# Ipsedo/MARLClassification

Hardware: NVIDIA B200
Metric: image_episodes_per_sec (higher is better)
Workload: dtype tf32x3

## Files before the change

marlclassification_b200/csrc/gemm_tc.cu:

```cuda
#include <cuda.h>
#include <stdlib.h>

#include "common.cuh"
#include "tc.cuh"

namespace marlc {

constexpr int BM = 128;
constexpr int BK = 32;
constexpr int UMMA_K = 8;
constexpr int TC_THREADS = 192;
constexpr int TC_THREADS_X3 = 320;
constexpr int TC_SPLITTERS = TC_THREADS_X3 - 64;
#define TC_SPLIT_GROUPS(stages) (((stages) % 2 == 0) ? 2 : 1)
constexpr int TC_MAX_CHAIN = 4096;

typedef CUresult (*EncodeTiledFn)(CUtensorMap*, CUtensorMapDataType, cuuint32_t, void*, const cuuint64_t*,
                                  const cuuint64_t*, const cuuint32_t*, const cuuint32_t*, CUtensorMapInterleave,
                                  CUtensorMapSwizzle, CUtensorMapL2promotion, CUtensorMapFloatOOBfill);
static EncodeTiledFn get_encode() {
    static EncodeTiledFn fn = nullptr;
    if (!fn) {
        void* p = nullptr;
        cudaDriverEntryPointQueryResult q;
        if (cudaGetDriverEntryPoint("cuTensorMapEncodeTiled", &p, cudaEnableDefault, &q) == cudaSuccess &&
            q == cudaDriverEntryPointSuccess)
            fn = (EncodeTiledFn)p;
    }
    return fn;
}

static int make_map(CUtensorMap* m, const float* ptr, long inner, long rows, long slabs, long ld, long slab_stride,
                    int box_rows, bool mn_major = false, int box_slabs = 1) {
    EncodeTiledFn enc = get_encode();
    MARLC_CHECK(enc, "cuTensorMapEncodeTiled not available");
    cuuint64_t dims[3] = {(cuuint64_t)inner, (cuuint64_t)rows, (cuuint64_t)slabs};
// ... 95 lines not shown
__device__ __forceinline__ float ex2_ftz(float x) { float y; asm("ex2.approx.ftz.f32 %0, %1;" : "=f"(y) : "f"(x)); return y; }
__device__ __forceinline__ float rcp_ftz(float x) { float y; asm("rcp.approx.ftz.f32 %0, %1;" : "=f"(y) : "f"(x)); return y; }
__device__ __forceinline__ float sigmoid_of_scaled(float t) { return rcp_ftz(1.0f + ex2_ftz(t)); }
__device__ __forceinline__ float tanh_of_scaled(float t) { return fmaf(2.0f, rcp_ftz(1.0f + ex2_ftz(t)), -1.0f); }
__device__ __forceinline__ float fast_tanh(float x) { return tanh_of_scaled(2.0f * NEG_LOG2E * x); }

__device__ __forceinline__ uint64_t make_desc(uint32_t saddr, uint32_t lbo_bytes, uint32_t sbo_bytes, uint32_t layout_type) {
    return (uint64_t)((saddr >> 4) & 0x3FFF) | ((uint64_t)((lbo_bytes >> 4) & 0x3FFF) << 16) |
           ((uint64_t)((sbo_bytes >> 4) & 0x3FFF) << 32) | (1ull << 46) | ((uint64_t)layout_type << 61);
}

enum { EPI_STORE = 0, EPI_LSTM = 1 };

struct TcKernelParams {
    CUtensorMap a1, b1, a2, b2;
    CUtensorMap a1l, b1l, a2l, b2l;
    CUtensorMap cmap;
    int c_tma;
    int ksplit;
    int a_lo_g, b_lo_g;
    int nk1, nk2;
    int slab_a1, slab_b1, slab_a2, slab_b2;
    int M, N;
    float* C;
    long ldc;
    const float* bias;
    const float* bias2;
    int accumulate, splits;
    const float* c_prev;
    float* c_new;
    float* h_new;
    float* h_new_lo;
    float* gates;
    int n_hidden;
};
constexpr int TC_MAX_GROUP = 3;
struct TcKernelGroup {
    TcKernelParams p[TC_MAX_GROUP];
    int zofs[TC_MAX_GROUP + 1];
    int count;
    int trig;
};

template <int BN, int STAGES, bool X3 = false, int KS = 1>
struct TcSmem {
    static constexpr int A_SUB = BM * BK * 4;
    static constexpr int B_SUB = BN * BK * 4;
    static constexpr int A_BYTES = KS * A_SUB;
    static constexpr int B_BYTES = KS * B_SUB;
    static constexpr int BYTES = STAGES * (A_BYTES + B_BYTES) * (X3 ? 2 : 1) + 1024;
};


template <int BN, bool A_MN, bool B_MN, int EPI, int STAGES, int PI, bool X3, int KS>
__device__ __forceinline__ void tc_gemm_body(const TcKernelGroup& pp, const int split) {
    using S = TcSmem<BN, STAGES, X3, KS>;
    extern __shared__ uint8_t smem_raw[];
    uint8_t* smem = (uint8_t*)(((uintptr_t)smem_raw + 1023) & ~(uintptr_t)1023);
    constexpr int stages = STAGES;
    uint8_t* sA = smem;
    uint8_t* sB = smem + stages * S::A_BYTES;
    constexpr int LO_OFF = stages * (S::A_BYTES + S::B_BYTES);
    __shared__ __align__(8) uint64_t full_bar[STAGES];
    __shared__ __align__(8) uint64_t empty_bar[STAGES];
    __shared__ __align__(8) uint64_t split_bar[STAGES];
    __shared__ __align__(8) uint64_t tmem_full_bar;
    __shared__ uint32_t tmem_base_smem;
    __shared__ float s_bias[8][BN];

    const TcKernelParams& p = pp.p[PI];
    const int warp = threadIdx.x >> 5, lane = threadIdx.x & 31;
#ifdef MARLC_TC_TRACE
    __shared__ long long trace[12];
    const bool tr = blockIdx.x == 0 && blockIdx.y == 0 && blockIdx.z == 0;
    const long long t_entry = clock64();
#define TC_TRACE(i) do { if (tr) trace[i] = clock64() - t_entry; } while (0)
#else
#define TC_TRACE(i) do { } while (0)
#endif
    const int m0 = blockIdx.y * BM;
    const int ksp = (EPI == EPI_LSTM && p.ksplit > 1) ? p.ksplit : 1;
    const int n_tile = ksp > 1 ? blockIdx.x / ksp : blockIdx.x;
    const int kslice = ksp > 1 ? blockIdx.x % ksp : 0;
    if (m0 >= p.M || n_tile * BN >= p.N) return;
    const int nkb = p.nk1 + p.nk2;
    int kb_begin = 0, kb_end = nkb;
    if (EPI == EPI_STORE && p.splits > 1) {
        const int per = (nkb + p.splits - 1) / p.splits;
        kb_begin = split * per;
        kb_end = min(nkb, kb_begin + per);
    }
    if (ksp > 1) {
        const int per = (nkb + ksp - 1) / ksp;
        kb_begin = kslice * per;
        kb_end = min(nkb, kb_begin + per);
    }
    const int my_kb = max(0, kb_end - kb_begin);
    constexpr int TMEM_COLS = BN < 32 ? 32 : BN;

    if (warp == 0 && lane == 0) {
        auto pf = [](const CUtensorMap* m) { asm volatile("prefetch.tensormap [%0];" ::"l"((uint64_t)m) : "memory"); };
        pf(&p.a1); pf(&p.b1);
        if (p.nk2 > 0) { pf(&p.a2); pf(&p.b2); }
        if (X3 && p.a_lo_g) { pf(&p.a1l); if (p.nk2 > 0) pf(&p.a2l); }
        if (X3 && p.b_lo_g) { pf(&p.b1l); if (p.nk2 > 0) pf(&p.b2l); }
        if (EPI == EPI_STORE && p.c_tma) pf(&p.cmap);
    }
    if (threadIdx.x == 32) {
        for (int s = 0; s < stages; ++s) {
            mbar_init(&full_bar[s], 1); mbar_init(&empty_bar[s], 1);
            mbar_init(&split_bar[s], TC_SPLITTERS / TC_SPLIT_GROUPS(STAGES));
        }
        mbar_init(&tmem_full_bar, 1);
        asm volatile("fence.mbarrier_init.release.cluster;" ::: "memory");
    }
    if (warp == 1) {
        asm volatile("tcgen05.alloc.cta_group::1.sync.aligned.shared::cta.b32 [%0], %1;" ::"r"(smem_u32(&tmem_base_smem)),
                     "r"(TMEM_COLS));
        asm volatile("tcgen05.relinquish_alloc_permit.cta_group::1.sync.aligned;");
    }
    tc_fence_before();
    __syncthreads();
    tc_fence_after();
    const uint32_t tmem_base = tmem_base_smem;
    pdl_wait();
    if (threadIdx.x == 0) TC_TRACE(0);
    if (ksp > 1) asm volatile("barrier.cluster.arrive.release;" ::: "memory");

    if (warp == 0) {
// ... 64 lines not shown
                    if (X3) {
                        const uint64_t lo = (uint64_t)((LO_OFF >> 4) & 0x3FFF);
                        umma_tf32(tmem_base, ad + lo, bd, idesc, 1u);
                        umma_tf32(tmem_base, ad, bd + lo, idesc, 1u);
                    }
                }
                }
                umma_commit(&empty_bar[s]);
            }
            umma_commit(&tmem_full_bar);
            TC_TRACE(3);
        }
    } else {
        const int q = warp & 3;
        const int m = m0 + 32 * q + lane;
        constexpr int HU_E = BN / 4;
        const bool epi8 = EPI == EPI_LSTM && X3 && HU_E >= 32 && ksp == 1 && p.a_lo_g && p.b_lo_g;
        const bool epi_warp = warp < 6 || epi8;
        const int jb_begin = (epi8 && warp >= 6) ? HU_E / 2 : 0;
        const int jb_end = epi8 ? (warp >= 6 ? HU_E : HU_E / 2) : HU_E;
        float cp_pref[8];
        if (epi_warp) {
            float* sb = s_bias[warp - 2];
            if (EPI == EPI_STORE) {
                const bool first_split0 = (p.splits <= 1) || (split == 0);
                for (int j = lane; j < BN; j += 32) {
                    const int n = n_tile * BN + j;
                    float b = 0.f;
                    if (first_split0 && n < p.N) {
                        if (p.bias) b += __ldg(p.bias + n);
                        if (p.bias2) b += __ldg(p.bias2 + n);
                    }
                    sb[j] = b;
                }
            } else {
                constexpr int HU = BN / 4;
                const int n = p.n_hidden, j0 = n_tile * HU;
                for (int j = lane; j < BN; j += 32) {
                    const int g = j / HU, col = g * n + j0 + (j - g * HU);
                    sb[j] = (__ldg(p.bias + col) + __ldg(p.bias2 + col)) * (g == 2 ? 2.0f * NEG_LOG2E : NEG_LOG2E);
                }
                if (m < p.M) {
                    const long off = (long)m * n + j0 + jb_begin;
                    const float4 c0 = *reinterpret_cast<const float4*>(p.c_prev + off);
                    const float4 c1 = *reinterpret_cast<const float4*>(p.c_prev + off + 4);
                    cp_pref[0] = c0.x; cp_pref[1] = c0.y; cp_pref[2] = c0.z; cp_pref[3] = c0.w;
                    cp_pref[4] = c1.x; cp_pref[5] = c1.y; cp_pref[6] = c1.z; cp_pref[7] = c1.w;
                }
            }
            __syncwarp();
        }
        if (X3) {
            constexpr int NGRP = TC_SPLIT_GROUPS(STAGES);
            constexpr int GRP = TC_SPLITTERS / NGRP;
            const int t = (threadIdx.x - 64) % GRP, grp = (threadIdx.x - 64) / GRP;
            const bool split_a = !p.a_lo_g, split_b = !p.b_lo_g;
            for (int i = grp; (split_a || split_b) && i < my_kb; i += NGRP) {
                const int s = i % stages, ph = (i / stages) & 1;
                mbar_wait(&full_bar[s], ph);
                float4* a_hi = reinterpret_cast<float4*>(sA + s * S::A_BYTES);
                float4* b_hi = reinterpret_cast<float4*>(sB + s * S::B_BYTES);
                float4* a_lo = reinterpret_cast<float4*>(sA + s * S::A_BYTES + LO_OFF);
                float4* b_lo = reinterpret_cast<float4*>(sB + s * S::B_BYTES + LO_OFF);
                auto lo_of = [](float x) { return x - __uint_as_float(__float_as_uint(x) & 0xFFFFE000u); };
#pragma unroll 4
                for (int v = t; split_a && v < S::A_BYTES / 16; v += GRP) {
                    const float4 x = a_hi[v];
                    a_lo[v] = make_float4(lo_of(x.x), lo_of(x.y), lo_of(x.z), lo_of(x.w));
                }
#pragma unroll 4
                for (int v = t; split_b && v < S::B_BYTES / 16; v += GRP) {
                    const float4 x = b_hi[v];
                    b_lo[v] = make_float4(lo_of(x.x), lo_of(x.y), lo_of(x.z), lo_of(x.w));
                }
                asm volatile("fence.proxy.async.shared::cta;" ::: "memory");
                asm volatile("mbarrier.arrive.shared::cta.b64 _, [%0];" ::"r"(smem_u32(&split_bar[s])) : "memory");
            }
        }
        if (epi_warp) {
        int e_M = p.M, e_N = p.N, e_mode = p.splits > 1 ? 2 : (p.accumulate ? 1 : 0);
        long e_ldc = p.ldc;
        float* e_C = p.C;
        asm volatile("" : "+r"(e_M), "+r"(e_N), "+r"(e_mode), "+l"(e_ldc), "+l"(e_C));
        mbar_wait(&tmem_full_bar, 0);
        tc_fence_after();
        if (warp == 2 && lane == 0) TC_TRACE(4);
        const uint32_t trow = tmem_base + ((uint32_t)(32 * q) << 16);
        if (EPI == EPI_STORE) {
            constexpr int PITCH = BN + 4;
            static_assert(EPI != EPI_STORE || 4 * 32 * PITCH * 4 <= S::BYTES - 1024, "epilogue staging tile does not fit in the ring");
            float* stg = reinterpret_cast<float*>(smem) + q * 32 * PITCH;
            const int nbase = n_tile * BN;
            const bool vec = ((e_ldc & 3) == 0) && (((uintptr_t)e_C & 15) == 0);
            if (p.c_tma) {
                constexpr int BOXES = BN / 32;
                const uint32_t box0 = smem_u32(smem) + (uint32_t)(q * BOXES) * 4096u;
#pragma unroll 1
                for (int c0 = 0; c0 < BN; c0 += 32) {
                    uint32_t r[32];
                    if (my_kb > 0) { TMEM_LD32(trow + c0, r); tmem_ld_wait(); }
                    else {
#pragma unroll
                        for (int j = 0; j < 32; ++j) r[j] = 0u;
                    }
                    const float* sb = s_bias[warp - 2] + c0;
                    const uint32_t rowb = box0 + (uint32_t)(c0 >> 5) * 4096u + (uint32_t)lane * 128u;
#pragma unroll
                    for (int j = 0; j < 32; j += 4) {
                        const uint32_t dst = rowb + (uint32_t)(((j >> 2) ^ (lane & 7)) << 4);
                        asm volatile("st.shared.v4.f32 [%0], {%1, %2, %3, %4};" ::"r"(dst),
                                     "f"(__uint_as_float(r[j]) + sb[j]), "f"(__uint_as_float(r[j + 1]) + sb[j + 1]),
                                     "f"(__uint_as_float(r[j + 2]) + sb[j + 2]), "f"(__uint_as_float(r[j + 3]) + sb[j + 3])
                                     : "memory");
                    }
                }
                asm volatile("fence.proxy.async.shared::cta;" ::: "memory");
                __syncwarp();
                if (warp == 2 && lane == 0) TC_TRACE(6);
                if (lane == 0 && m0 + 32 * q < e_M) {
#pragma unroll 1
                    for (int b = 0; b < BOXES; ++b) {
                        const int cn = nbase + 32 * b;
                        if (cn >= e_N) break;
                        const uint32_t src = box0 + (uint32_t)b * 4096u;
                        if (e_mode == 0)
                            asm volatile("cp.async.bulk.tensor.2d.global.shared::cta.bulk_group [%0, {%2, %3}], [%1];" ::"l"(
                                             (uint64_t)&p.cmap), "r"(src), "r"(cn), "r"(m0 + 32 * q) : "memory");
                        else
                            asm volatile("cp.reduce.async.bulk.tensor.2d.global.shared::cta.add.tile.bulk_group [%0, {%2, %3}], [%1];" ::"l"(
                                             (uint64_t)&p.cmap), "r"(src), "r"(cn), "r"(m0 + 32 * q) : "memory");
                    }
                    asm volatile("cp.async.bulk.commit_group;" ::: "memory");
                    asm volatile("cp.async.bulk.wait_group.read 0;" ::: "memory");
                }
            } else {
            const uint32_t stg_s = smem_u32(stg);
#pragma unroll 1
            for (int c0 = 0; c0 < BN; c0 += 32) {
                uint32_t r[32];
                if (my_kb > 0) { TMEM_LD32(trow + c0, r); tmem_ld_wait(); }
                else {
#pragma unroll
                    for (int j = 0; j < 32; ++j) r[j] = 0u;
                }
                const float* sb = s_bias[warp - 2] + c0;
#pragma unroll
                for (int j = 0; j < 32; j += 4) {
                    const float4 v = make_float4(__uint_as_float(r[j]) + sb[j], __uint_as_float(r[j + 1]) + sb[j + 1],
                                                 __uint_as_float(r[j + 2]) + sb[j + 2], __uint_as_float(r[j + 3]) + sb[j + 3]);
                    asm volatile("st.shared.v4.f32 [%0], {%1, %2, %3, %4};" ::"r"(stg_s + (uint32_t)(lane * PITCH + c0 + j) * 4),
                                 "f"(v.x), "f"(v.y), "f"(v.z), "f"(v.w) : "memory");
                }
            }
            __syncwarp();
            constexpr int LPR = BN / 4;
            constexpr int RPI = 32 / LPR;
            const int rr = lane / LPR, c4 = (lane % LPR) * 4;
            const int n = nbase + c4;
            const bool full4 = vec && n + 4 <= e_N;
            if (n < e_N) {
#pragma unroll 1
                for (int r0 = 0; r0 < 32; r0 += RPI) {
                    const int row = r0 + rr, mrow = m0 + 32 * q + row;
                    if (mrow >= e_M) break;
                    float4 v;
                    asm volatile("ld.shared.v4.f32 {%0, %1, %2, %3}, [%4];" : "=f"(v.x), "=f"(v.y), "=f"(v.z), "=f"(v.w)
                                 : "r"(stg_s + (uint32_t)(row * PITCH + c4) * 4));
                    float* crow = e_C + (long)mrow * e_ldc + n;
#ifdef MARLC_TC_NOSTORE
                    if (v.x == 123.456f) crow[0] = v.y;
                    continue;
#endif
#ifdef MARLC_TC_TRACE
                    if (warp == 2 && lane == 0 && r0 == RPI * 2) TC_TRACE(7);
#endif
                    if (full4) {
                        if (e_mode == 2) {
                            atomicAdd(reinterpret_cast<float4*>(crow), v);
                        } else {
                            if (e_mode == 1) {
                                const float4 o = *reinterpret_cast<const float4*>(crow);
                                v.x += o.x; v.y += o.y; v.z += o.z; v.w += o.w;
                            }
                            *reinterpret_cast<float4*>(crow) = v;
                        }
                    } else {
                        const float vv[4] = {v.x, v.y, v.z, v.w};
#pragma unroll
                        for (int j = 0; j < 4; ++j) {
                            if (n + j >= e_N) break;
                            if (e_mode == 2) atomicAdd(crow + j, vv[j]);
                            else crow[j] = e_mode == 1 ? crow[j] + vv[j] : vv[j];
                        }
                    }
                }
            }
            }
        } else {
            constexpr int HU = BN / 4;
            const int n = p.n_hidden, j0 = n_tile * HU;
            constexpr int PPITCH = BN + 4;
            float* part = reinterpret_cast<float*>(smem + (S::BYTES - 1024));
            if (ksp > 1) asm volatile("barrier.cluster.wait.acquire;" ::: "memory");
            if (ksp > 1 && kslice != 0) {
                uint32_t remote;
                asm volatile("mapa.shared::cluster.u32 %0, %1, %2;" : "=r"(remote) : "r"(smem_u32(part)), "r"(0));
                const uint32_t rrow = remote + (uint32_t)((32 * q + lane) * PPITCH) * 4u;
#pragma unroll 1
                for (int c0 = 0; c0 < BN; c0 += 8) {
                    uint32_t r[8];
                    if (my_kb > 0) { TMEM_LD8(trow + c0, r); tmem_ld_wait(); }
                    else {
#pragma unroll
                        for (int j = 0; j < 8; ++j) r[j] = 0u;
                    }
                    asm volatile("st.shared::cluster.v4.b32 [%0], {%1, %2, %3, %4};" ::"r"(rrow + (uint32_t)c0 * 4u), "r"(r[0]),
                                 "r"(r[1]), "r"(r[2]), "r"(r[3]) : "memory");
                    asm volatile("st.shared::cluster.v4.b32 [%0], {%1, %2, %3, %4};" ::"r"(rrow + (uint32_t)c0 * 4u + 16u), "r"(r[4]),
                                 "r"(r[5]), "r"(r[6]), "r"(r[7]) : "memory");
                }
            }
// ... 103 lines not shown
                    }
                    __syncwarp();
#ifdef MARLC_TC_TRACE
                    if (warp == 2 && lane == 0 && jb + 8 == CH) TC_TRACE(9);
#endif
                }
            }
            }
        }
        }
    }
    if (ksp > 1 && !(warp >= 2 && warp < 6)) {
        asm volatile("barrier.cluster.wait.acquire;" ::: "memory");
        asm volatile("barrier.cluster.arrive.release;" ::: "memory");
        asm volatile("barrier.cluster.wait.acquire;" ::: "memory");
    }
    if (warp == 2 && lane == 0) TC_TRACE(5);
    tc_fence_before();
    __syncthreads();
#ifdef MARLC_TC_TRACE
    if (tr && threadIdx.x == 0)
        printf("tc trace BN=%d X3=%d KS=%d EPI=%d kb=%d: setup %lld | tma0 %lld | full0 %lld | mma_issued %lld | acc_done %lld | epi_done %lld | end %lld\n",
               BN, (int)X3, KS, EPI, my_kb, trace[0], trace[1], trace[2], trace[3], trace[4], trace[5], clock64() - t_entry);
    if (tr && threadIdx.x == 0 && EPI == EPI_STORE) printf("   staged at %lld, third store iteration at %lld\n", trace[6], trace[7]);
    if (tr && threadIdx.x == 0 && EPI == EPI_LSTM)
        printf("   cell: first 8 units loaded %lld | activated %lld | staged %lld | second 8 staged %lld | first chunk written out %lld\n",
               trace[6], trace[7], trace[8], trace[10], trace[9]);
#endif
    if (warp == 1) {
        tc_fence_after();
        asm volatile("tcgen05.dealloc.cta_group::1.sync.aligned.b32 %0, %1;" ::"r"(tmem_base), "r"(TMEM_COLS));
    }
}

template <int BN, bool A_MN, bool B_MN, int EPI, int STAGES, bool X3, int KS>
__global__ void __launch_bounds__(X3 ? TC_THREADS_X3 : TC_THREADS, 1) tc_gemm_kernel(const __grid_constant__ TcKernelGroup pp) {
    if (pp.trig) pdl_trigger();
    const int z = blockIdx.z;
    if (pp.count >= 3 && z >= pp.zofs[2]) tc_gemm_body<BN, A_MN, B_MN, EPI, STAGES, 2, X3, KS>(pp, z - pp.zofs[2]);
    else if (pp.count >= 2 && z >= pp.zofs[1]) tc_gemm_body<BN, A_MN, B_MN, EPI, STAGES, 1, X3, KS>(pp, z - pp.zofs[1]);
    else tc_gemm_body<BN, A_MN, B_MN, EPI, STAGES, 0, X3, KS>(pp, z);
}

static int operand_map(CUtensorMap* m, const TcOperand& o, int mn_extent, int k_extent, int box_rows_kmajor) {
    if (!o.mn_major) return make_map(m, o.ptr, k_extent, mn_extent, o.slabs, o.ld, o.slab_stride, box_rows_kmajor);
    return make_map(m, o.ptr, mn_extent, k_extent, o.slabs, o.ld, o.slab_stride, 32, true);
}

template <int BN, bool A_MN, bool B_MN, bool X3, int KS>
static int launch_store(TcKernelGroup& kp, int gx, int gy, int gz, int max_kb, cudaStream_t s) {
    (void)max_kb;
    constexpr int STAGES = KS > 1 ? 2 : (BN >= 128 ? 3 : 4);
    using S = TcSmem<BN, STAGES, X3, KS>;
    static_assert(S::BYTES <= 227 * 1024, "tile configuration exceeds shared memory");
    auto kern = tc_gemm_kernel<BN, A_MN, B_MN, EPI_STORE, STAGES, X3, KS>;
    static bool attr_done = false;
    if (!attr_done) {
        MARLC_CUDA(cudaFuncSetAttribute(kern, cudaFuncAttributeMaxDynamicSharedMemorySize, S::BYTES));
        attr_done = true;
    }
    kp.trig = pdl_trigger_early();
    MARLC_CUDA(launch_pdl(kern, dim3(gx, gy, gz), dim3(X3 ? TC_THREADS_X3 : TC_THREADS), S::BYTES, s, kp));
    ++g_tc_gemm_launches;
    MARLC_LAUNCH_CHECK();
    return 0;
}

constexpr int TC_DX128_MIN_CTAS = 16;
static int pick_bn(const TcGemmArgs* args, int count) {
    int max_n = 0;
    long ctas128 = 0;
    for (int i = 0; i < count; ++i) {
        const TcGemmArgs& a = args[i];
        max_n = max(max_n, a.N);
        long chains = a.allow_split ? max(1L, ((long)a.K + a.K2 + TC_MAX_CHAIN - 1) / TC_MAX_CHAIN) : 1L;
        if (a.allow_split == 1 && a.A.mn_major && a.B.mn_major) chains = max(chains, ((long)a.K + a.K2) / 128);
        ctas128 += (long)((a.M + BM - 1) / BM) * ((a.N + 127) / 128) * chains;
    }
    if (max_n <= 32) return 32;
    const bool dx_group = !args[0].A.mn_major && args[0].B.mn_major && count > 1;
    if (max_n <= 64 || ctas128 < (dx_group ? TC_DX128_MIN_CTAS : MARLC_SMS / 2)) return 64;
    return 128;
}

int tc_gemm_group(const TcGemmArgs* args, int count, cudaStream_t s) {
    MARLC_CHECK(count >= 1 && count <= TC_MAX_GROUP, "tc_gemm_group: count=%d", count);
    const int BN = pick_bn(args, count);
    TcKernelGroup kp;
    memset(&kp, 0, sizeof(kp));
    kp.count = count;
    int gx = 0, gy = 0, ctas = 0, min_k = 1 << 30;
    int pdl_ok = g_pdl;
    for (int i = 0; i < count; ++i) {
        const TcGemmArgs& a = args[i];
        ctas += ((a.M + BM - 1) / BM) * ((a.N + BN - 1) / BN);
        min_k = min(min_k, a.K + a.K2);
    }
    const int KS = (ctas < MARLC_SMS && BN <= 64 && min_k >= 128) ? 2 : 1;
    const int BKS = BK * KS;
    for (int i = 0; i < count; ++i) {
        const TcGemmArgs& a = args[i];
        MARLC_CHECK(tc_operand_ok(a.A) && tc_operand_ok(a.B), "tc_gemm: operand not TMA-addressable");
        MARLC_CHECK(a.K > 0 && a.M > 0 && a.N > 0, "tc_gemm: empty problem");
        MARLC_CHECK(a.A.mn_major == args[0].A.mn_major && a.B.mn_major == args[0].B.mn_major,
                    "tc_gemm_group: all problems must share operand majors");
        const bool pair2 = a.K2 > 0;
        if (pair2) {
            MARLC_CHECK(tc_operand_ok(a.A2) && tc_operand_ok(a.B2), "tc_gemm: second operand pair not TMA-addressable");
            MARLC_CHECK(a.A2.mn_major == a.A.mn_major && a.B2.mn_major == a.B.mn_major, "tc_gemm: operand pairs must share majors");
        }
        TcKernelParams& p = kp.p[i];
        MARLC_TRY(operand_map(&p.a1, a.A, a.M, a.K, BM));
        MARLC_TRY(operand_map(&p.b1, a.B, a.N, a.K, BN));
        p.nk1 = (a.K + BKS - 1) / BKS;
        p.slab_a1 = a.A.slab; p.slab_b1 = a.B.slab;
        p.a_lo_g = (a.x3 && a.A.lo && (!pair2 || a.A2.lo)) ? 1 : 0;
        p.b_lo_g = (a.x3 && a.B.lo && (!pair2 || a.B2.lo)) ? 1 : 0;
        if (p.a_lo_g) { TcOperand o = a.A; o.ptr = a.A.lo; MARLC_TRY(operand_map(&p.a1l, o, a.M, a.K, BM)); }
        if (p.b_lo_g) { TcOperand o = a.B; o.ptr = a.B.lo; MARLC_TRY(operand_map(&p.b1l, o, a.N, a.K, BN)); }
        if (pair2) {
            MARLC_TRY(operand_map(&p.a2, a.A2, a.M, a.K2, BM));
            MARLC_TRY(operand_map(&p.b2, a.B2, a.N, a.K2, BN));
            p.nk2 = (a.K2 + BKS - 1) / BKS;
            p.slab_a2 = a.A2.slab; p.slab_b2 = a.B2.slab;
            if (p.a_lo_g) { TcOperand o = a.A2; o.ptr = a.A2.lo; MARLC_TRY(operand_map(&p.a2l, o, a.M, a.K2, BM)); }
            if (p.b_lo_g) { TcOperand o = a.B2; o.ptr = a.B2.lo; MARLC_TRY(operand_map(&p.b2l, o, a.N, a.K2, BN)); }
        }
        p.M = a.M; p.N = a.N; p.C = a.C; p.ldc = a.ldc; p.bias = a.bias; p.bias2 = a.bias2;
        p.accumulate = a.accumulate;
        p.c_tma = ((a.ldc & 3) == 0 && ((uintptr_t)a.C & 15) == 0) ? 1 : 0;
        if (p.c_tma) MARLC_TRY(make_map_c(&p.cmap, a.C, a.M, a.N, a.ldc));
        const int mt = (a.M + BM - 1) / BM, nt = (a.N + BN - 1) / BN, nkb = p.nk1 + p.nk2;
        int splits = 1;
        if (a.allow_split && ctas < MARLC_SMS) {
            splits = min(a.allow_split >= 2 ? nkb : max(1, nkb * KS / 4), max(1, MARLC_SMS / ctas));
            splits = min(splits, nkb);
        }
        if (a.allow_split) {
            const int chain_blocks = max(1, TC_MAX_CHAIN / BKS);
            splits = max(splits, (nkb + chain_blocks - 1) / chain_blocks);
            while (splits > 1 && ((nkb + splits - 1) / splits) * (splits - 1) >= nkb) --splits;
        }
        p.splits = splits;
        if (splits > 1 && !a.accumulate && !a.c_zeroed) {
            pdl_ok = 0;
            if (a.ldc == a.N) MARLC_CUDA(cudaMemsetAsync(a.C, 0, sizeof(float) * (size_t)a.M * a.N, s));
            else MARLC_CUDA(cudaMemset2DAsync(a.C, sizeof(float) * a.ldc, 0, sizeof(float) * a.N, a.M, s));
        }
        kp.zofs[i + 1] = kp.zofs[i] + splits;
        gx = max(gx, nt);
        gy = max(gy, mt);
    }
    const int gz = kp.zofs[count];
    PdlScope pdl_scope(pdl_ok, g_pdl_trig);
    int max_kb = 1;
    for (int i = 0; i < count; ++i) {
        const int nkb = kp.p[i].nk1 + kp.p[i].nk2;
        max_kb = max(max_kb, (nkb + kp.p[i].splits - 1) / kp.p[i].splits);
    }
    const bool amn = args[0].A.mn_major, bmn = args[0].B.mn_major;
    const bool x3 = args[0].x3 != 0;
#define DISPATCH3(BNv, X, KSv)                                                                   \
    if (amn) {                                                                                   \
        if (bmn) return launch_store<BNv, true, true, X, KSv>(kp, gx, gy, gz, max_kb, s);        \
        return launch_store<BNv, true, false, X, KSv>(kp, gx, gy, gz, max_kb, s);                \
    } else {                                                                                     \
        if (bmn) return launch_store<BNv, false, true, X, KSv>(kp, gx, gy, gz, max_kb, s);       \
        return launch_store<BNv, false, false, X, KSv>(kp, gx, gy, gz, max_kb, s);               \
    }
#define DISPATCH(BNv, KSv)            \
    if (x3) { DISPATCH3(BNv, true, KSv) } \
    else { DISPATCH3(BNv, false, KSv) }
    if (BN == 32) { if (KS == 2) { DISPATCH(32, 2) } DISPATCH(32, 1) }
    if (BN == 64) { if (KS == 2) { DISPATCH(64, 2) } DISPATCH(64, 1) }
    DISPATCH(128, 1)
#undef DISPATCH
#undef DISPATCH3
}

int tc_gemm(const TcGemmArgs& a, cudaStream_t s) { return tc_gemm_group(&a, 1, s); }

template <int BN, bool X3, int KS>
static int launch_lstm(TcKernelGroup& kp, int gx, int gy, int nkb, cudaStream_t s) {
    (void)nkb;
    constexpr int STAGES = BN >= 256 ? (X3 ? 2 : 4) : (KS > 1 ? 2 : (BN >= 128 ? 3 : 4));
    using S = TcSmem<BN, STAGES, X3, KS>;
    static_assert(S::BYTES <= 227 * 1024, "tile configuration exceeds shared memory");
    auto kern = tc_gemm_kernel<BN, false, false, EPI_LSTM, STAGES, X3, KS>;
    static bool attr_done = false;
    if (!attr_done) {
        MARLC_CUDA(cudaFuncSetAttribute(kern, cudaFuncAttributeMaxDynamicSharedMemorySize, S::BYTES));
// ... 107 lines not shown
```

Before: 20090.

## Make store GEMM a persistent kernel with double-buffered TMEM accumulators

Splits the plain-store tcgen05 GEMM into its own persistent kernel body. The grid is capped at the resident CTA count, and each CTA walks a flat list of (group, split, tile) units. Two TMEM accumulators with full/empty barriers and a dedicated staging buffer let one tile's epilogue overlap the next tile's TMA and MMA, and the x3 path gets extra threads. This removes per-tile launch, prologue and epilogue serialization, but the kernel grows more complex, uses more shared memory and twice the TMEM columns, and forces lo-operand flags to be uniform across the group.

```diff
diff --git a/marlclassification_b200/csrc/gemm_tc.cu b/marlclassification_b200/csrc/gemm_tc.cu
--- a/marlclassification_b200/csrc/gemm_tc.cu
+++ b/marlclassification_b200/csrc/gemm_tc.cu
@@ -12,6 +12,8 @@
 constexpr int TC_THREADS = 192;
 constexpr int TC_THREADS_X3 = 320;
 constexpr int TC_SPLITTERS = TC_THREADS_X3 - 64;
+constexpr int TC_STORE_THREADS_X3 = TC_THREADS + TC_SPLITTERS;
+constexpr int TC_STG_BYTES = 4 * 2 * 4096;
 #define TC_SPLIT_GROUPS(stages) (((stages) % 2 == 0) ? 2 : 1)
 constexpr int TC_MAX_CHAIN = 4096;
 
@@ -153,6 +155,7 @@
     int nk1, nk2;
     int slab_a1, slab_b1, slab_a2, slab_b2;
     int M, N;
+    int mt, nt;
     float* C;
     long ldc;
     const float* bias;
@@ -184,7 +187,8 @@
 
 
 template <int BN, bool A_MN, bool B_MN, int EPI, int STAGES, int PI, bool X3, int KS>
-__device__ __forceinline__ void tc_gemm_body(const TcKernelGroup& pp, const int split) {
+__device__ __forceinline__ void tc_gemm_body(const TcKernelGroup& pp) {
+    static_assert(EPI == EPI_LSTM, "EPI_STORE runs on tc_store_body");
     using S = TcSmem<BN, STAGES, X3, KS>;
     extern __shared__ uint8_t smem_raw[];
     uint8_t* smem = (uint8_t*)(((uintptr_t)smem_raw + 1023) & ~(uintptr_t)1023);
@@ -216,11 +220,6 @@
     if (m0 >= p.M || n_tile * BN >= p.N) return;
     const int nkb = p.nk1 + p.nk2;
     int kb_begin = 0, kb_end = nkb;
-    if (EPI == EPI_STORE && p.splits > 1) {
-        const int per = (nkb + p.splits - 1) / p.splits;
-        kb_begin = split * per;
-        kb_end = min(nkb, kb_begin + per);
-    }
     if (ksp > 1) {
         const int per = (nkb + ksp - 1) / ksp;
         kb_begin = kslice * per;
@@ -235,7 +234,6 @@
         if (p.nk2 > 0) { pf(&p.a2); pf(&p.b2); }
         if (X3 && p.a_lo_g) { pf(&p.a1l); if (p.nk2 > 0) pf(&p.a2l); }
         if (X3 && p.b_lo_g) { pf(&p.b1l); if (p.nk2 > 0) pf(&p.b2l); }
-        if (EPI == EPI_STORE && p.c_tma) pf(&p.cmap);
     }
     if (threadIdx.x == 32) {
         for (int s = 0; s < stages; ++s) {
@@ -346,18 +344,7 @@
         float cp_pref[8];
         if (epi_warp) {
             float* sb = s_bias[warp - 2];
-            if (EPI == EPI_STORE) {
-                const bool first_split0 = (p.splits <= 1) || (split == 0);
-                for (int j = lane; j < BN; j += 32) {
-                    const int n = n_tile * BN + j;
-                    float b = 0.f;
-                    if (first_split0 && n < p.N) {
-                        if (p.bias) b += __ldg(p.bias + n);
-                        if (p.bias2) b += __ldg(p.bias2 + n);
-                    }
-                    sb[j] = b;
-                }
-            } else {
+            {
                 constexpr int HU = BN / 4;
                 const int n = p.n_hidden, j0 = n_tile * HU;
                 for (int j = lane; j < BN; j += 32) {
@@ -402,125 +389,11 @@
             }
         }
         if (epi_warp) {
-        int e_M = p.M, e_N = p.N, e_mode = p.splits > 1 ? 2 : (p.accumulate ? 1 : 0);
-        long e_ldc = p.ldc;
-        float* e_C = p.C;
-        asm volatile("" : "+r"(e_M), "+r"(e_N), "+r"(e_mode), "+l"(e_ldc), "+l"(e_C));
         mbar_wait(&tmem_full_bar, 0);
         tc_fence_after();
         if (warp == 2 && lane == 0) TC_TRACE(4);
         const uint32_t trow = tmem_base + ((uint32_t)(32 * q) << 16);
-        if (EPI == EPI_STORE) {
-            constexpr int PITCH = BN + 4;
-            static_assert(EPI != EPI_STORE || 4 * 32 * PITCH * 4 <= S::BYTES - 1024, "epilogue staging tile does not fit in the ring");
-            float* stg = reinterpret_cast<float*>(smem) + q * 32 * PITCH;
-            const int nbase = n_tile * BN;
-            const bool vec = ((e_ldc & 3) == 0) && (((uintptr_t)e_C & 15) == 0);
-            if (p.c_tma) {
-                constexpr int BOXES = BN / 32;
-                const uint32_t box0 = smem_u32(smem) + (uint32_t)(q * BOXES) * 4096u;
-#pragma unroll 1
-                for (int c0 = 0; c0 < BN; c0 += 32) {
-                    uint32_t r[32];
-                    if (my_kb > 0) { TMEM_LD32(trow + c0, r); tmem_ld_wait(); }
-                    else {
-#pragma unroll
-                        for (int j = 0; j < 32; ++j) r[j] = 0u;
-                    }
-                    const float* sb = s_bias[warp - 2] + c0;
-                    const uint32_t rowb = box0 + (uint32_t)(c0 >> 5) * 4096u + (uint32_t)lane * 128u;
-#pragma unroll
-                    for (int j = 0; j < 32; j += 4) {
-                        const uint32_t dst = rowb + (uint32_t)(((j >> 2) ^ (lane & 7)) << 4);
-                        asm volatile("st.shared.v4.f32 [%0], {%1, %2, %3, %4};" ::"r"(dst),
-                                     "f"(__uint_as_float(r[j]) + sb[j]), "f"(__uint_as_float(r[j + 1]) + sb[j + 1]),
-                                     "f"(__uint_as_float(r[j + 2]) + sb[j + 2]), "f"(__uint_as_float(r[j + 3]) + sb[j + 3])
-                                     : "memory");
-                    }
-                }
-                asm volatile("fence.proxy.async.shared::cta;" ::: "memory");
-                __syncwarp();
-                if (warp == 2 && lane == 0) TC_TRACE(6);
-                if (lane == 0 && m0 + 32 * q < e_M) {
-#pragma unroll 1
-                    for (int b = 0; b < BOXES; ++b) {
-                        const int cn = nbase + 32 * b;
-                        if (cn >= e_N) break;
-                        const uint32_t src = box0 + (uint32_t)b * 4096u;
-                        if (e_mode == 0)
-                            asm volatile("cp.async.bulk.tensor.2d.global.shared::cta.bulk_group [%0, {%2, %3}], [%1];" ::"l"(
-                                             (uint64_t)&p.cmap), "r"(src), "r"(cn), "r"(m0 + 32 * q) : "memory");
-                        else
-                            asm volatile("cp.reduce.async.bulk.tensor.2d.global.shared::cta.add.tile.bulk_group [%0, {%2, %3}], [%1];" ::"l"(
-                                             (uint64_t)&p.cmap), "r"(src), "r"(cn), "r"(m0 + 32 * q) : "memory");
-                    }
-                    asm volatile("cp.async.bulk.commit_group;" ::: "memory");
-                    asm volatile("cp.async.bulk.wait_group.read 0;" ::: "memory");
-                }
-            } else {
-            const uint32_t stg_s = smem_u32(stg);
-#pragma unroll 1
-            for (int c0 = 0; c0 < BN; c0 += 32) {
-                uint32_t r[32];
-                if (my_kb > 0) { TMEM_LD32(trow + c0, r); tmem_ld_wait(); }
-                else {
-#pragma unroll
-                    for (int j = 0; j < 32; ++j) r[j] = 0u;
-                }
-                const float* sb = s_bias[warp - 2] + c0;
-#pragma unroll
-                for (int j = 0; j < 32; j += 4) {
-                    const float4 v = make_float4(__uint_as_float(r[j]) + sb[j], __uint_as_float(r[j + 1]) + sb[j + 1],
-                                                 __uint_as_float(r[j + 2]) + sb[j + 2], __uint_as_float(r[j + 3]) + sb[j + 3]);
-                    asm volatile("st.shared.v4.f32 [%0], {%1, %2, %3, %4};" ::"r"(stg_s + (uint32_t)(lane * PITCH + c0 + j) * 4),
-                                 "f"(v.x), "f"(v.y), "f"(v.z), "f"(v.w) : "memory");
-                }
-            }
-            __syncwarp();
-            constexpr int LPR = BN / 4;
-            constexpr int RPI = 32 / LPR;
-            const int rr = lane / LPR, c4 = (lane % LPR) * 4;
-            const int n = nbase + c4;
-            const bool full4 = vec && n + 4 <= e_N;
-            if (n < e_N) {
-#pragma unroll 1
-                for (int r0 = 0; r0 < 32; r0 += RPI) {
-                    const int row = r0 + rr, mrow = m0 + 32 * q + row;
-                    if (mrow >= e_M) break;
-                    float4 v;
-                    asm volatile("ld.shared.v4.f32 {%0, %1, %2, %3}, [%4];" : "=f"(v.x), "=f"(v.y), "=f"(v.z), "=f"(v.w)
-                                 : "r"(stg_s + (uint32_t)(row * PITCH + c4) * 4));
-                    float* crow = e_C + (long)mrow * e_ldc + n;
-#ifdef MARLC_TC_NOSTORE
-                    if (v.x == 123.456f) crow[0] = v.y;
-                    continue;
-#endif
-#ifdef MARLC_TC_TRACE
-                    if (warp == 2 && lane == 0 && r0 == RPI * 2) TC_TRACE(7);
-#endif
-                    if (full4) {
-                        if (e_mode == 2) {
-                            atomicAdd(reinterpret_cast<float4*>(crow), v);
-                        } else {
-                            if (e_mode == 1) {
-                                const float4 o = *reinterpret_cast<const float4*>(crow);
-                                v.x += o.x; v.y += o.y; v.z += o.z; v.w += o.w;
-                            }
-                            *reinterpret_cast<float4*>(crow) = v;
-                        }
-                    } else {
-                        const float vv[4] = {v.x, v.y, v.z, v.w};
-#pragma unroll
-                        for (int j = 0; j < 4; ++j) {
-                            if (n + j >= e_N) break;
-                            if (e_mode == 2) atomicAdd(crow + j, vv[j]);
-                            else crow[j] = e_mode == 1 ? crow[j] + vv[j] : vv[j];
-                        }
-                    }
-                }
-            }
-            }
-        } else {
+        {
             constexpr int HU = BN / 4;
             const int n = p.n_hidden, j0 = n_tile * HU;
             constexpr int PPITCH = BN + 4;
@@ -670,8 +543,7 @@
     if (tr && threadIdx.x == 0)
         printf("tc trace BN=%d X3=%d KS=%d EPI=%d kb=%d: setup %lld | tma0 %lld | full0 %lld | mma_issued %lld | acc_done %lld | epi_done %lld | end %lld\n",
                BN, (int)X3, KS, EPI, my_kb, trace[0], trace[1], trace[2], trace[3], trace[4], trace[5], clock64() - t_entry);
-    if (tr && threadIdx.x == 0 && EPI == EPI_STORE) printf("   staged at %lld, third store iteration at %lld\n", trace[6], trace[7]);
-    if (tr && threadIdx.x == 0 && EPI == EPI_LSTM)
+    if (tr && threadIdx.x == 0)
         printf("   cell: first 8 units loaded %lld | activated %lld | staged %lld | second 8 staged %lld | first chunk written out %lld\n",
                trace[6], trace[7], trace[8], trace[10], trace[9]);
 #endif
@@ -681,13 +553,371 @@
     }
 }
 
+struct TcUnit {
+    uint64_t a1, b1, a2, b2, a1l, b1l, a2l, b2l, cmap;
+    const float* bias;
+    const float* bias2;
+    float* C;
+    long ldc;
+    int m0, n0, kb_begin, nkb, nk1, za1, za2, zb1, zb2, a_lo, b_lo, M, N, mode, c_tma, first_split;
+};
+
+template <int PI, int BN>
+__device__ __forceinline__ TcUnit tc_unit_of(const TcKernelGroup& pp, int u) {
+    const TcKernelParams& p = pp.p[PI];
+    const int tiles = p.mt * p.nt;
+    const int split = u / tiles, r = u - split * tiles;
+    const int mt = r / p.nt;
+    TcUnit x;
+    x.a1 = (uint64_t)&p.a1; x.b1 = (uint64_t)&p.b1; x.a2 = (uint64_t)&p.a2; x.b2 = (uint64_t)&p.b2;
+    x.a1l = (uint64_t)&p.a1l; x.b1l = (uint64_t)&p.b1l; x.a2l = (uint64_t)&p.a2l; x.b2l = (uint64_t)&p.b2l;
+    x.cmap = (uint64_t)&p.cmap;
+    x.bias = p.bias; x.bias2 = p.bias2; x.C = p.C; x.ldc = p.ldc;
+    x.m0 = mt * BM;
+    x.n0 = (r - mt * p.nt) * BN;
+    const int nkb = p.nk1 + p.nk2;
+    x.kb_begin = 0;
+    int kb_end = nkb;
+    if (p.splits > 1) {
+        const int per = (nkb + p.splits - 1) / p.splits;
+        x.kb_begin = split * per;
+        kb_end = min(nkb, x.kb_begin + per);
+    }
+    x.nkb = max(0, kb_end - x.kb_begin);
+    x.nk1 = p.nk1;
+    x.za1 = p.slab_a1; x.za2 = p.slab_a2; x.zb1 = p.slab_b1; x.zb2 = p.slab_b2;
+    x.a_lo = p.a_lo_g; x.b_lo = p.b_lo_g;
+    x.M = p.M; x.N = p.N;
+    x.mode = p.splits > 1 ? 2 : (p.accumulate ? 1 : 0);
+    x.c_tma = p.c_tma;
+    x.first_split = split == 0;
+    return x;
+}
+template <int BN>
+__device__ __forceinline__ TcUnit tc_unit_at(const TcKernelGroup& pp, int u) {
+    if (pp.count >= 3 && u >= pp.zofs[2]) return tc_unit_of<2, BN>(pp, u - pp.zofs[2]);
+    if (pp.count >= 2 && u >= pp.zofs[1]) return tc_unit_of<1, BN>(pp, u - pp.zofs[1]);
+    return tc_unit_of<0, BN>(pp, u);
+}
+
+template <int BN, bool A_MN, bool B_MN, int STAGES, bool X3, int KS>
+__device__ __forceinline__ void tc_store_body(const TcKernelGroup& pp) {
+    using S = TcSmem<BN, STAGES, X3, KS>;
+    extern __shared__ uint8_t smem_raw[];
+    uint8_t* smem = (uint8_t*)(((uintptr_t)smem_raw + 1023) & ~(uintptr_t)1023);
+    constexpr int RING = S::BYTES - 1024;
+    uint8_t* sA = smem;
+    uint8_t* sB = smem + STAGES * S::A_BYTES;
+    constexpr int LO_OFF = STAGES * (S::A_BYTES + S::B_BYTES);
+    __shared__ __align__(8) uint64_t full_bar[STAGES];
+    __shared__ __align__(8) uint64_t empty_bar[STAGES];
+    __shared__ __align__(8) uint64_t split_bar[STAGES];
+    __shared__ __align__(8) uint64_t tmem_full_bar[2];
+    __shared__ __align__(8) uint64_t tmem_empty_bar[2];
+    __shared__ uint32_t tmem_base_smem;
+    constexpr int TMEM_COLS = 2 * BN < 32 ? 32 : 2 * BN;
+    static_assert(2 * BN <= 256, "two accumulators of a persistent CTA must leave TMEM for a second CTA on the SM");
+
+    const int warp = threadIdx.x >> 5, lane = threadIdx.x & 31;
+    const int units = pp.zofs[pp.count];
+#undef TC_TRACE
+#ifdef MARLC_TC_TRACE
+    __shared__ long long trace[8];
+    const bool tr = blockIdx.x == 0;
+    const long long t_entry = clock64();
+#define TC_TRACE(i) do { if (tr) trace[i] = clock64() - t_entry; } while (0)
+#else
+#define TC_TRACE(i) do { } while (0)
+#endif
+
+    if (warp == 0 && lane == 0 && (int)blockIdx.x < units) {
+        const TcUnit x = tc_unit_at<BN>(pp, blockIdx.x);
+        auto pf = [](uint64_t m) { asm volatile("prefetch.tensormap [%0];" ::"l"(m) : "memory"); };
+        pf(x.a1); pf(x.b1);
+        if (x.nk1 < x.kb_begin + x.nkb) { pf(x.a2); pf(x.b2); }
+        if (X3 && x.a_lo) pf(x.a1l);
+        if (X3 && x.b_lo) pf(x.b1l);
+        if (x.c_tma) pf(x.cmap);
+    }
+    if (threadIdx.x == 32) {
+        for (int s = 0; s < STAGES; ++s) {
+            mbar_init(&full_bar[s], 1); mbar_init(&empty_bar[s], 1);
+            mbar_init(&split_bar[s], TC_SPLITTERS / TC_SPLIT_GROUPS(STAGES));
+        }
+        for (int a = 0; a < 2; ++a) { mbar_init(&tmem_full_bar[a], 1); mbar_init(&tmem_empty_bar[a], 4); }
+        asm volatile("fence.mbarrier_init.release.cluster;" ::: "memory");
+    }
+    if (warp == 1) {
+        asm volatile("tcgen05.alloc.cta_group::1.sync.aligned.shared::cta.b32 [%0], %1;" ::"r"(smem_u32(&tmem_base_smem)),
+                     "r"(TMEM_COLS));
+        asm volatile("tcgen05.relinquish_alloc_permit.cta_group::1.sync.aligned;");
+    }
+    tc_fence_before();
+    __syncthreads();
+    tc_fence_after();
+    const uint32_t tmem_base = tmem_base_smem;
+    pdl_wait();
+    if (threadIdx.x == 0) TC_TRACE(0);
+
+    if (warp == 0) {
+        if (lane == 0) {
+            uint32_t g = 0;
+            for (int u = blockIdx.x; u < units; u += gridDim.x) {
+                const TcUnit x = tc_unit_at<BN>(pp, u);
+                const int q_alo = X3 ? x.a_lo : 0, q_blo = X3 ? x.b_lo : 0;
+                const uint32_t tx_bytes = S::A_BYTES + S::B_BYTES + (q_alo ? S::A_BYTES : 0) + (q_blo ? S::B_BYTES : 0);
+                for (int i = 0; i < x.nkb; ++i, ++g) {
+                    const int s = g % STAGES, ph = (g / STAGES) & 1;
+                    mbar_wait(&empty_bar[s], ph ^ 1);
+                    mbar_expect_tx(&full_bar[s], tx_bytes);
+                    const int kb = x.kb_begin + i;
+                    const bool second = kb >= x.nk1;
+                    const int za = second ? x.za2 : x.za1, zb = second ? x.zb2 : x.zb1;
+                    const int nlo = X3 ? 2 : 1;
+                    for (int hl = 0; hl < nlo; ++hl) {
+                        if (hl == 1 && !q_alo && !q_blo) break;
+                        const CUtensorMap* ma = (const CUtensorMap*)(hl ? (second ? x.a2l : x.a1l) : (second ? x.a2 : x.a1));
+                        const CUtensorMap* mb = (const CUtensorMap*)(hl ? (second ? x.b2l : x.b1l) : (second ? x.b2 : x.b1));
+                        const bool do_a = hl == 0 || q_alo, do_b = hl == 0 || q_blo;
+#pragma unroll
+                        for (int sub = 0; sub < KS; ++sub) {
+                            const int k0 = ((second ? kb - x.nk1 : kb) * KS + sub) * BK;
+                            uint8_t* a_dst = sA + s * S::A_BYTES + sub * S::A_SUB + hl * LO_OFF;
+                            uint8_t* b_dst = sB + s * S::B_BYTES + sub * S::B_SUB + hl * LO_OFF;
+                            if (do_a) {
+                                if (!A_MN) tma_load_3d(a_dst, ma, &full_bar[s], k0, x.m0, za);
+                                else
+                                    for (int j = 0; j < BM / 32; ++j) tma_load_3d(a_dst + j * 4096, ma, &full_bar[s], x.m0 + 32 * j, k0, za);
+                            }
+                            if (!do_b) continue;
+                            if (!B_MN) tma_load_3d(b_dst, mb, &full_bar[s], k0, x.n0, zb);
+                            else
+                                for (int j = 0; j < BN / 32; ++j) tma_load_3d(b_dst + j * 4096, mb, &full_bar[s], x.n0 + 32 * j, k0, zb);
+                        }
+                    }
+                    if (g == 0) TC_TRACE(1);
+                }
+            }
+        }
+    } else if (warp == 1) {
+        if (lane == 0) {
+            constexpr uint32_t idesc = (1u << 4) | (2u << 7) | (2u << 10) | ((A_MN ? 1u : 0u) << 15) |
+                                       ((B_MN ? 1u : 0u) << 16) | ((uint32_t)(BN >> 3) << 17) | ((uint32_t)(BM >> 4) << 24);
+            uint32_t g = 0, t = 0;
+            for (int u = blockIdx.x; u < units; u += gridDim.x, ++t) {
+                const TcUnit x = tc_unit_at<BN>(pp, u);
+                const bool wait_split = X3 && !(x.a_lo && x.b_lo);
+                const uint32_t as = t & 1;
+                mbar_wait(&tmem_empty_bar[as], ((t >> 1) & 1) ^ 1);
+                tc_fence_after();
+                const uint32_t acc = tmem_base + as * BN;
+                for (int i = 0; i < x.nkb; ++i, ++g) {
+                    const int s = g % STAGES, ph = (g / STAGES) & 1;
+                    mbar_wait(wait_split ? &split_bar[s] : &full_bar[s], ph);
+                    tc_fence_after();
+                    if (g == 0) TC_TRACE(2);
+#pragma unroll
+                    for (int sub = 0; sub < KS; ++sub) {
+                        const uint32_t a_addr = smem_u32(sA + s * S::A_BYTES + sub * S::A_SUB);
+                        const uint32_t b_addr = smem_u32(sB + s * S::B_BYTES + sub * S::B_SUB);
+#pragma unroll
+                        for (int k = 0; k < BK / UMMA_K; ++k) {
+                            const uint64_t ad = A_MN ? make_desc(a_addr + k * 1024, 4096, 512, 1) : make_desc(a_addr + k * 32, 16, 1024, 2);
+                            const uint64_t bd = B_MN ? make_desc(b_addr + k * 1024, 4096, 512, 1) : make_desc(b_addr + k * 32, 16, 1024, 2);
+                            umma_tf32(acc, ad, bd, idesc, (i > 0 || k > 0 || sub > 0) ? 1u : 0u);
+                            if (X3) {
+                                const uint64_t lo = (uint64_t)((LO_OFF >> 4) & 0x3FFF);
+                                umma_tf32(acc, ad + lo, bd, idesc, 1u);
+                                umma_tf32(acc, ad, bd + lo, idesc, 1u);
+                            }
+                        }
+                    }
+                    umma_commit(&empty_bar[s]);
+                }
+                umma_commit(&tmem_full_bar[as]);
+                if (t == 0) TC_TRACE(3);
+            }
+        }
+    } else if (warp >= 6) {
+        if (X3) {
+            constexpr int NGRP = TC_SPLIT_GROUPS(STAGES);
+            constexpr int GRP = TC_SPLITTERS / NGRP;
+            const int tid = (threadIdx.x - TC_THREADS) % GRP, grp = (threadIdx.x - TC_THREADS) / GRP;
+            uint32_t g = 0;
+            for (int u = blockIdx.x; u < units; u += gridDim.x) {
+                const TcUnit x = tc_unit_at<BN>(pp, u);
+                const bool split_a = !x.a_lo, split_b = !x.b_lo;
+                for (int i = 0; (split_a || split_b) && i < x.nkb; ++i) {
+                    const uint32_t gi = g + i;
+                    if ((int)(gi % NGRP) != grp) continue;
+                    const int s = gi % STAGES, ph = (gi / STAGES) & 1;
+                    mbar_wait(&full_bar[s], ph);
+                    float4* a_hi = reinterpret_cast<float4*>(sA + s * S::A_BYTES);
+                    float4* b_hi = reinterpret_cast<float4*>(sB + s * S::B_BYTES);
+                    float4* a_lo = reinterpret_cast<float4*>(sA + s * S::A_BYTES + LO_OFF);
+                    float4* b_lo = reinterpret_cast<float4*>(sB + s * S::B_BYTES + LO_OFF);
+                    auto lo_of = [](float v) { return v - __uint_as_float(__float_as_uint(v) & 0xFFFFE000u); };
+#pragma unroll 4
+                    for (int v = tid; split_a && v < S::A_BYTES / 16; v += GRP) {
+                        const float4 y = a_hi[v];
+                        a_lo[v] = make_float4(lo_of(y.x), lo_of(y.y), lo_of(y.z), lo_of(y.w));
+                    }
+#pragma unroll 4
+                    for (int v = tid; split_b && v < S::B_BYTES / 16; v += GRP) {
+                        const float4 y = b_hi[v];
+                        b_lo[v] = make_float4(lo_of(y.x), lo_of(y.y), lo_of(y.z), lo_of(y.w));
+                    }
+                    asm volatile("fence.proxy.async.shared::cta;" ::: "memory");
+                    asm volatile("mbarrier.arrive.shared::cta.b64 _, [%0];" ::"r"(smem_u32(&split_bar[s])) : "memory");
+                }
+                g += x.nkb;
+            }
+        }
+    } else {
+        const int q = warp & 3;
+        const uint32_t stg0 = smem_u32(smem + RING) + (uint32_t)(warp - 2) * 8192u;
+        uint32_t t = 0, chunk = 0;
+        for (int u = blockIdx.x; u < units; u += gridDim.x, ++t) {
+            const TcUnit x = tc_unit_at<BN>(pp, u);
+            float bias_r[(BN + 31) / 32];
+#pragma unroll
+            for (int c = 0; c < (BN + 31) / 32; ++c) {
+                const int n = x.n0 + 32 * c + lane;
+                float b = 0.f;
+                if (x.first_split && n < x.N) {
+                    if (x.bias) b += __ldg(x.bias + n);
+                    if (x.bias2) b += __ldg(x.bias2 + n);
+                }
+                bias_r[c] = b;
+            }
+            const uint32_t as = t & 1;
+            mbar_wait(&tmem_full_bar[as], (t >> 1) & 1);
+            tc_fence_after();
+            if (t == 0 && warp == 2 && lane == 0) TC_TRACE(4);
+            const uint32_t trow = tmem_base + ((uint32_t)(32 * q) << 16) + as * BN;
+            const int row0 = x.m0 + 32 * q;
+#pragma unroll
+            for (int c = 0; c < BN / 32; ++c, ++chunk) {
+                uint32_t r[32];
+                if (x.nkb > 0) { TMEM_LD32(trow + 32 * c, r); tmem_ld_wait(); }
+                else {
+#pragma unroll
+                    for (int j = 0; j < 32; ++j) r[j] = 0u;
+                }
+                if (c == BN / 32 - 1) {
+                    tc_fence_before();
+                    __syncwarp();
+                    if (lane == 0) asm volatile("mbarrier.arrive.shared::cta.b64 _, [%0];" ::"r"(smem_u32(&tmem_empty_bar[as])) : "memory");
+                }
+                const int cn = x.n0 + 32 * c;
+                if (x.c_tma) {
+                    const uint32_t box = stg0 + (chunk & 1) * 4096u;
+                    if (lane == 0) asm volatile("cp.async.bulk.wait_group.read 1;" ::: "memory");
+                    __syncwarp();
+                    const uint32_t rowb = box + (uint32_t)lane * 128u;
+#pragma unroll
+                    for (int j = 0; j < 32; j += 4) {
+                        const uint32_t dst = rowb + (uint32_t)(((j >> 2) ^ (lane & 7)) << 4);
+                        asm volatile("st.shared.v4.f32 [%0], {%1, %2, %3, %4};" ::"r"(dst),
+                                     "f"(__uint_as_float(r[j]) + __shfl_sync(0xffffffffu, bias_r[c], j)),
+                                     "f"(__uint_as_float(r[j + 1]) + __shfl_sync(0xffffffffu, bias_r[c], j + 1)),
+                                     "f"(__uint_as_float(r[j + 2]) + __shfl_sync(0xffffffffu, bias_r[c], j + 2)),
+                                     "f"(__uint_as_float(r[j + 3]) + __shfl_sync(0xffffffffu, bias_r[c], j + 3))
+                                     : "memory");
+                    }
+                    asm volatile("fence.proxy.async.shared::cta;" ::: "memory");
+                    __syncwarp();
+                    if (lane == 0) {
+                        if (row0 < x.M && cn < x.N) {
+                            if (x.mode == 0)
+                                asm volatile("cp.async.bulk.tensor.2d.global.shared::cta.bulk_group [%0, {%2, %3}], [%1];" ::"l"(
+                                                 x.cmap), "r"(box), "r"(cn), "r"(row0) : "memory");
+                            else
+                                asm volatile("cp.reduce.async.bulk.tensor.2d.global.shared::cta.add.tile.bulk_group [%0, {%2, %3}], [%1];" ::"l"(
+                                                 x.cmap), "r"(box), "r"(cn), "r"(row0) : "memory");
+                        }
+                        asm volatile("cp.async.bulk.commit_group;" ::: "memory");
+                    }
+                } else {
+                    constexpr int PITCH = 32 + 4;
+                    if (lane == 0) asm volatile("cp.async.bulk.wait_group.read 0;" ::: "memory");
+                    __syncwarp();
+#pragma unroll
+                    for (int j = 0; j < 32; j += 4) {
+                        asm volatile("st.shared.v4.f32 [%0], {%1, %2, %3, %4};" ::"r"(stg0 + (uint32_t)(lane * PITCH + j) * 4),
+                                     "f"(__uint_as_float(r[j]) + __shfl_sync(0xffffffffu, bias_r[c], j)),
+                                     "f"(__uint_as_float(r[j + 1]) + __shfl_sync(0xffffffffu, bias_r[c], j + 1)),
+                                     "f"(__uint_as_float(r[j + 2]) + __shfl_sync(0xffffffffu, bias_r[c], j + 2)),
+                                     "f"(__uint_as_float(r[j + 3]) + __shfl_sync(0xffffffffu, bias_r[c], j + 3))
+                                     : "memory");
+                    }
+                    __syncwarp();
+                    const int rr = lane >> 3, c4 = (lane & 7) * 4;
+                    const int n = cn + c4;
+                    const bool full4 = ((x.ldc & 3) == 0) && (((uintptr_t)x.C & 15) == 0) && n + 4 <= x.N;
+                    if (n < x.N) {
+#pragma unroll 1
+                        for (int r0 = 0; r0 < 32; r0 += 4) {
+                            const int row = r0 + rr, mrow = row0 + row;
+                            if (mrow >= x.M) break;
+                            float4 v;
+                            asm volatile("ld.shared.v4.f32 {%0, %1, %2, %3}, [%4];" : "=f"(v.x), "=f"(v.y), "=f"(v.z), "=f"(v.w)
+                                         : "r"(stg0 + (uint32_t)(row * PITCH + c4) * 4));
+                            float* crow = x.C + (long)mrow * x.ldc + n;
+                            if (full4) {
+                                if (x.mode == 2) {
+                                    atomicAdd(reinterpret_cast<float4*>(crow), v);
+                                } else {
+                                    if (x.mode == 1) {
+                                        const float4 o = *reinterpret_cast<const float4*>(crow);
+                                        v.x += o.x; v.y += o.y; v.z += o.z; v.w += o.w;
+                                    }
+                                    *reinterpret_cast<float4*>(crow) = v;
+                                }
+                            } else {
+                                const float vv[4] = {v.x, v.y, v.z, v.w};
+#pragma unroll
+                                for (int j = 0; j < 4; ++j) {
+                                    if (n + j >= x.N) break;
+                                    if (x.mode == 2) atomicAdd(crow + j, vv[j]);
+                                    else crow[j] = x.mode == 1 ? crow[j] + vv[j] : vv[j];
+                                }
+                            }
+                        }
+                    }
+                    __syncwarp();
+                }
+            }
+            if (t == 0 && warp == 2 && lane == 0) TC_TRACE(5);
+        }
+        if (lane == 0) asm volatile("cp.async.bulk.wait_group.read 0;" ::: "memory");
+    }
+    tc_fence_before();
+    __syncthreads();
+#ifdef MARLC_TC_TRACE
+    if (tr && threadIdx.x == 0)
+        printf("tc trace BN=%d X3=%d KS=%d EPI=0 units=%d grid=%d: setup %lld | tma0 %lld | full0 %lld | mma_issued %lld | acc_done %lld | epi_done %lld | end %lld\n",
+               BN, (int)X3, KS, units, (int)gridDim.x, trace[0], trace[1], trace[2], trace[3], trace[4], trace[5], clock64() - t_entry);
+#endif
+#undef TC_TRACE
+    if (warp == 1) {
+        tc_fence_after();
+        asm volatile("tcgen05.dealloc.cta_group::1.sync.aligned.b32 %0, %1;" ::"r"(tmem_base), "r"(TMEM_COLS));
+    }
+}
+
 template <int BN, bool A_MN, bool B_MN, int EPI, int STAGES, bool X3, int KS>
-__global__ void __launch_bounds__(X3 ? TC_THREADS_X3 : TC_THREADS, 1) tc_gemm_kernel(const __grid_constant__ TcKernelGroup pp) {
+__global__ void __launch_bounds__(X3 ? (EPI == EPI_STORE ? TC_STORE_THREADS_X3 : TC_THREADS_X3) : TC_THREADS, 1)
+    tc_gemm_kernel(const __grid_constant__ TcKernelGroup pp) {
     if (pp.trig) pdl_trigger();
-    const int z = blockIdx.z;
-    if (pp.count >= 3 && z >= pp.zofs[2]) tc_gemm_body<BN, A_MN, B_MN, EPI, STAGES, 2, X3, KS>(pp, z - pp.zofs[2]);
-    else if (pp.count >= 2 && z >= pp.zofs[1]) tc_gemm_body<BN, A_MN, B_MN, EPI, STAGES, 1, X3, KS>(pp, z - pp.zofs[1]);
-    else tc_gemm_body<BN, A_MN, B_MN, EPI, STAGES, 0, X3, KS>(pp, z);
+    if constexpr (EPI == EPI_STORE) {
+        tc_store_body<BN, A_MN, B_MN, STAGES, X3, KS>(pp);
+    } else {
+        const int z = blockIdx.z;
+        if (pp.count >= 3 && z >= pp.zofs[2]) tc_gemm_body<BN, A_MN, B_MN, EPI, STAGES, 2, X3, KS>(pp);
+        else if (pp.count >= 2 && z >= pp.zofs[1]) tc_gemm_body<BN, A_MN, B_MN, EPI, STAGES, 1, X3, KS>(pp);
+        else tc_gemm_body<BN, A_MN, B_MN, EPI, STAGES, 0, X3, KS>(pp);
+    }
 }
 
 static int operand_map(CUtensorMap* m, const TcOperand& o, int mn_extent, int k_extent, int box_rows_kmajor) {
@@ -696,19 +926,23 @@
 }
 
 template <int BN, bool A_MN, bool B_MN, bool X3, int KS>
-static int launch_store(TcKernelGroup& kp, int gx, int gy, int gz, int max_kb, cudaStream_t s) {
-    (void)max_kb;
-    constexpr int STAGES = KS > 1 ? 2 : (BN >= 128 ? 3 : 4);
+static int launch_store(TcKernelGroup& kp, int units, cudaStream_t s) {
+    constexpr int STAGES = KS > 1 ? 2 : (X3 ? (BN >= 128 ? 3 : 4) : (BN >= 128 ? 2 : 3));
     using S = TcSmem<BN, STAGES, X3, KS>;
-    static_assert(S::BYTES <= 227 * 1024, "tile configuration exceeds shared memory");
+    constexpr int SMEM = S::BYTES + TC_STG_BYTES;
+    static_assert(SMEM <= 227 * 1024 - 256, "tile configuration exceeds shared memory");
+    constexpr int THREADS = X3 ? TC_STORE_THREADS_X3 : TC_THREADS;
     auto kern = tc_gemm_kernel<BN, A_MN, B_MN, EPI_STORE, STAGES, X3, KS>;
-    static bool attr_done = false;
-    if (!attr_done) {
-        MARLC_CUDA(cudaFuncSetAttribute(kern, cudaFuncAttributeMaxDynamicSharedMemorySize, S::BYTES));
-        attr_done = true;
+    static int resident = 0;
+    if (!resident) {
+        MARLC_CUDA(cudaFuncSetAttribute(kern, cudaFuncAttributeMaxDynamicSharedMemorySize, SMEM));
+        int per_sm = 0;
+        MARLC_CUDA(cudaOccupancyMaxActiveBlocksPerMultiprocessor(&per_sm, kern, THREADS, SMEM));
+        MARLC_CHECK(per_sm >= 1, "tc_gemm: kernel cannot be resident (BN=%d, %d bytes of shared memory)", BN, SMEM);
+        resident = per_sm * MARLC_SMS;
     }
     kp.trig = pdl_trigger_early();
-    MARLC_CUDA(launch_pdl(kern, dim3(gx, gy, gz), dim3(X3 ? TC_THREADS_X3 : TC_THREADS), S::BYTES, s, kp));
+    MARLC_CUDA(launch_pdl(kern, dim3(min(units, resident)), dim3(THREADS), SMEM, s, kp));
     ++g_tc_gemm_launches;
     MARLC_LAUNCH_CHECK();
     return 0;
@@ -737,12 +971,14 @@
     TcKernelGroup kp;
     memset(&kp, 0, sizeof(kp));
     kp.count = count;
-    int gx = 0, gy = 0, ctas = 0, min_k = 1 << 30;
+    int ctas = 0, min_k = 1 << 30, a_lo_all = 1, b_lo_all = 1;
     int pdl_ok = g_pdl;
     for (int i = 0; i < count; ++i) {
         const TcGemmArgs& a = args[i];
         ctas += ((a.M + BM - 1) / BM) * ((a.N + BN - 1) / BN);
         min_k = min(min_k, a.K + a.K2);
+        if (!(a.x3 && a.A.lo && (a.K2 == 0 || a.A2.lo))) a_lo_all = 0;
+        if (!(a.x3 && a.B.lo && (a.K2 == 0 || a.B2.lo))) b_lo_all = 0;
     }
     const int KS = (ctas < MARLC_SMS && BN <= 64 && min_k >= 128) ? 2 : 1;
     const int BKS = BK * KS;
@@ -762,8 +998,8 @@
         MARLC_TRY(operand_map(&p.b1, a.B, a.N, a.K, BN));
         p.nk1 = (a.K + BKS - 1) / BKS;
         p.slab_a1 = a.A.slab; p.slab_b1 = a.B.slab;
-        p.a_lo_g = (a.x3 && a.A.lo && (!pair2 || a.A2.lo)) ? 1 : 0;
-        p.b_lo_g = (a.x3 && a.B.lo && (!pair2 || a.B2.lo)) ? 1 : 0;
+        p.a_lo_g = a_lo_all;
+        p.b_lo_g = b_lo_all;
         if (p.a_lo_g) { TcOperand o = a.A; o.ptr = a.A.lo; MARLC_TRY(operand_map(&p.a1l, o, a.M, a.K, BM)); }
         if (p.b_lo_g) { TcOperand o = a.B; o.ptr = a.B.lo; MARLC_TRY(operand_map(&p.b1l, o, a.N, a.K, BN)); }
         if (pair2) {
@@ -795,26 +1031,20 @@
             if (a.ldc == a.N) MARLC_CUDA(cudaMemsetAsync(a.C, 0, sizeof(float) * (size_t)a.M * a.N, s));
             else MARLC_CUDA(cudaMemset2DAsync(a.C, sizeof(float) * a.ldc, 0, sizeof(float) * a.N, a.M, s));
         }
-        kp.zofs[i + 1] = kp.zofs[i] + splits;
-        gx = max(gx, nt);
-        gy = max(gy, mt);
-    }
-    const int gz = kp.zofs[count];
+        p.mt = mt; p.nt = nt;
+        kp.zofs[i + 1] = kp.zofs[i] + splits * mt * nt;
+    }
+    const int units = kp.zofs[count];
     PdlScope pdl_scope(pdl_ok, g_pdl_trig);
-    int max_kb = 1;
-    for (int i = 0; i < count; ++i) {
-        const int nkb = kp.p[i].nk1 + kp.p[i].nk2;
-        max_kb = max(max_kb, (nkb + kp.p[i].splits - 1) / kp.p[i].splits);
-    }
     const bool amn = args[0].A.mn_major, bmn = args[0].B.mn_major;
     const bool x3 = args[0].x3 != 0;
 #define DISPATCH3(BNv, X, KSv)                                                                   \
     if (amn) {                                                                                   \
-        if (bmn) return launch_store<BNv, true, true, X, KSv>(kp, gx, gy, gz, max_kb, s);        \
-        return launch_store<BNv, true, false, X, KSv>(kp, gx, gy, gz, max_kb, s);                \
+        if (bmn) return launch_store<BNv, true, true, X, KSv>(kp, units, s);        \
+        return launch_store<BNv, true, false, X, KSv>(kp, units, s);                \
     } else {                                                                                     \
-        if (bmn) return launch_store<BNv, false, true, X, KSv>(kp, gx, gy, gz, max_kb, s);       \
-        return launch_store<BNv, false, false, X, KSv>(kp, gx, gy, gz, max_kb, s);               \
+        if (bmn) return launch_store<BNv, false, true, X, KSv>(kp, units, s);       \
+        return launch_store<BNv, false, false, X, KSv>(kp, units, s);               \
     }
 #define DISPATCH(BNv, KSv)            \
     if (x3) { DISPATCH3(BNv, true, KSv) } \
```

After: 20410, median of 6. 1.02x the previous value.
